# ToddThomson/Mila

Hardware: AMD Instinct MI355X
Metric: Gemma-4 12B decode tok/s (B=1, context 2048), 1xMI355X (higher is better)
Workload: dtype bf16; 1 GPU; Gemma-4 12B, weight policy bf16, B=1, prefill T=2048 then decode at positions 2048..; decode_mode=graph, replicas=1, parallelism=replicas only (no collective), bounded_local_kv=0

## Files before the change

include/mila_cdna4.h:

```cpp
#ifndef MILA_CDNA4_H
#define MILA_CDNA4_H

#include <stddef.h>
#include <stdint.h>

#ifdef __cplusplus
extern "C" {
#endif

#if defined(__GNUC__)
#define MILA_API __attribute__((visibility("default")))
#else
#define MILA_API
#endif

typedef void* mila_stream_t;

enum {
    MILA_OK = 0,
    MILA_E_INVALID_ARGUMENT = -1,
    MILA_E_UNSUPPORTED = -2,
    MILA_E_RUNTIME = -3,
    MILA_E_SCRATCH_TOO_SMALL = -4
};
// ... 215 lines not shown
    int* argmax_blocks;
} mila_fused_matvec_args;
MILA_API int mila_cdna4_fused_norm_matvec(const mila_fused_matvec_args* host_args, mila_stream_t stream);

MILA_API int mila_cdna4_fused_qkv_post(uint16_t* q_out, uint16_t* Kc, uint16_t* Vc, const uint16_t* q,
                                       const uint16_t* k, const uint16_t* v_src, const uint16_t* qw,
                                       const uint16_t* kw, const uint16_t* vw, const float* cos_cache,
                                       const float* sin_cache, int NH, int NKV, int HS, int position,
                                       int capacity, float eps, mila_stream_t stream);


MILA_API int mila_cdna4_fused_qkv_post_prefill(uint16_t* q_out, uint16_t* Kc, uint16_t* Vc, const uint16_t* q,
                                               const uint16_t* k, const uint16_t* v_src, int64_t src_row_stride,
                                               const uint16_t* qw, const uint16_t* kw, const uint16_t* vw,
                                               const float* cos_cache, const float* sin_cache, int T, int NH, int NKV,
                                               int HS, int pos_offset, int capacity, float eps, mila_stream_t stream);
MILA_API int mila_cdna4_fused_tail_norm_bf16(uint16_t* R, uint16_t* XN, const uint16_t* A, const uint16_t* RES,
                                             const uint16_t* post_w, const uint16_t* next_w, int rows, int dim,
                                             float post_scale, float eps, mila_stream_t stream);
MILA_API int mila_cdna4_fused_tail_norm_quant_bf16(uint16_t* R, uint16_t* XN, uint8_t* XQ, float* XS, const uint16_t* A,
                                                   const uint16_t* RES, const uint16_t* post_w, const uint16_t* next_w, int rows,
                                                   int dim, float post_scale, float eps, mila_stream_t stream);

MILA_API int mila_cdna4_attn_decode_bf16_devpos(uint16_t* Y, const uint16_t* Q, const uint16_t* Kc,
                                                const uint16_t* Vc, void* scratch, size_t scratch_bytes,
                                                int B, int NH, int NKV, int HS, int capacity,
                                                const int32_t* position_dev, int max_len, int window,
                                                float scale, mila_stream_t stream);
MILA_API int mila_cdna4_fused_qkv_post_devpos(uint16_t* q_out, uint16_t* Kc, uint16_t* Vc, const uint16_t* q,
                                              const uint16_t* k, const uint16_t* v_src, const uint16_t* qw,
                                              const uint16_t* kw, const uint16_t* vw, const float* cos_cache,
                                              const float* sin_cache, int NH, int NKV, int HS,
                                              const int32_t* position_dev, int capacity, float eps,
                                              mila_stream_t stream);
MILA_API int mila_cdna4_advance_position(int32_t* position_dev, mila_stream_t stream);
MILA_API int mila_cdna4_advance_position_snapshot(int32_t* position_dev, const int32_t* token, unsigned long long* seq_dev, unsigned long long* ring, int ring_size,
                                                  mila_stream_t stream);
MILA_API int mila_cdna4_snapshot_token(const int32_t* token, unsigned long long* seq_dev, unsigned long long* ring, int ring_size, mila_stream_t stream);
MILA_API int mila_cdna4_sample_argmax_advance_fp32(const float* logits, int32_t* token_out, int vocab, void* scratch, size_t scratch_bytes,
                                                   int32_t* position_dev, unsigned long long* seq_dev, unsigned long long* ring, int ring_size,
                                                   mila_stream_t stream);

MILA_API int mila_cdna4_sample_argmax_final_advance(int32_t* token_out, const void* scratch, size_t scratch_bytes, int blocks, int32_t* position_dev,
                                                    unsigned long long* seq_dev, unsigned long long* ring, int ring_size, mila_stream_t stream);

MILA_API int mila_cdna4_fused_attn_decode_bf16(uint16_t* Y, uint16_t* Kc, uint16_t* Vc, const uint16_t* q_raw,
                                               const uint16_t* k_raw, const uint16_t* v_raw, const uint16_t* qw,
                                               const uint16_t* kw, const uint16_t* vw, const float* cos_cache,
                                               const float* sin_cache, void* scratch, size_t scratch_bytes, int NH,
                                               int NKV, int HS, int capacity, int position,
                                               const int32_t* position_dev, int window, float scale, float eps,
                                               mila_stream_t stream);

MILA_API int mila_cdna4_fused_attn_decode_batch_bf16(uint16_t* Y, uint16_t* Kc, uint16_t* Vc, const uint16_t* q_raw, const uint16_t* k_raw,
                                                     const uint16_t* v_raw, int64_t raw_b_stride, const uint16_t* qw, const uint16_t* kw,
                                                     const uint16_t* vw, const float* cos_cache, const float* sin_cache, void* scratch,
                                                     size_t scratch_bytes, int B, int NH, int NKV, int HS, int capacity, int position,
                                                     const int32_t* position_dev, int window, float scale, float eps, mila_stream_t stream);

#ifdef __cplusplus
}
#endif
#endif
```

mila_amd/capi.py:

```python
import ctypes as C
import os

_HERE = os.path.dirname(os.path.abspath(__file__))
LIB_PATH = os.path.join(_HERE, "lib", "libmila_cdna4.so")

MILA_OK = 0
MILA_E_INVALID_ARGUMENT = -1
MILA_E_UNSUPPORTED = -2
MILA_E_RUNTIME = -3
MILA_E_SCRATCH_TOO_SMALL = -4

FMT_BF16, FMT_FP8, FMT_FP4 = 0, 1, 2


class MilaError(RuntimeError):
    def __init__(self, code, text):
        super().__init__("mila_cdna4 error %d: %s" % (code, text))
        self.code = code


class InvalidArgument(MilaError, ValueError):
    """reference: std::invalid_argument"""


# ... 104 lines not shown
    lib = load()
    lib.mila_cdna4_gemm_plan_describe.restype = C.c_size_t
    buf = C.create_string_buffer(8192)
    need = lib.mila_cdna4_gemm_plan_describe(PLAN_ENTRIES.index(entry) if isinstance(entry, str) else int(entry), int(M), int(K), int(N), buf, C.c_size_t(len(buf)))
    assert need <= len(buf), "plan text of %d bytes" % need
    return [(f[0],) + tuple(int(v) for v in f[1:]) for f in (item.split(":") for item in buf.value.decode().split("+") if item)]


def check(rc):
    if rc == MILA_OK:
        return
    text = load().mila_cdna4_last_error().decode()
    if rc == MILA_E_INVALID_ARGUMENT:
        raise InvalidArgument(rc, text)
    raise MilaError(rc, text)


def call(name, *args):
    fn = getattr(load(), "mila_cdna4_" + name)
    conv = []
    for a in args:
        if a is None or isinstance(a, (C.c_void_p, C.c_float, C.c_int, C.c_int64, C.c_size_t)):
            conv.append(a)
        elif isinstance(a, float):
            conv.append(C.c_float(a))
        elif isinstance(a, int):
            conv.append(C.c_int(a))
        elif hasattr(a, "data_ptr"):
            conv.append(_ptr(a))
        else:
            conv.append(a)
    check(fn(*conv, _stream()))


EXPORTED = [
    "last_error", "abi_version", "device_count", "set_device", "device_info", "stream_create",
    "stream_destroy", "stream_synchronize", "malloc", "free", "host_alloc_pinned", "host_free_pinned",
    "memcpy_h2d", "memcpy_d2h", "memcpy_d2d", "memset_zero",
    "matvec_bf16", "matvec_bf16_qfp8", "matvec_bf16_qfp4", "matvec_f32out",
    "gemm_bf16", "gemm_gelu_bf16", "gemm_workspace_bytes", "gemm_bf16_ws", "gemm_bf16_w8a16", "gemm_bf16_w4a16", "gemm_staging_bytes", "gemm_bf16_w8a16_staged", "gemm_bf16_w4a16_staged",
    "fp4_weight_fp8_scale", "upcast_fp4_to_fp8", "quantize_fp8_per_token", "gemm_fp8_applicable", "gemm_fp8_scaled", "gemm_fp8_workspace_bytes", "gemm_fp8_scaled_ws",
    "gemm_w4a8_scratch_bytes", "gemm_bf16_w4a8", "gemm_geglu_w4a8_applicable", "gemm_geglu_bf16_w4a8",
    "gemm_geglu_applicable", "gemm_geglu_preferred", "gemm_geglu_bf16", "gemm_geglu_bf16_w8a16_staged", "gemm_geglu_bf16_w4a16_staged",
    "quantize_fp8_per_channel", "quantize_fp4_per_group",
    "kv_write_bf16", "attn_decode_scratch_bytes", "attn_decode_bf16", "attn_prefill_bf16", "mha_bf16", "mha_kv_write_bf16", "mha_decode_scratch_bytes", "mha_decode_bf16",
    "rmsnorm_bf16", "rmsnorm_fp32", "layernorm_bf16", "layernorm_fp32", "softmax_fp32", "softmax_bf16",
    "gelu_bf16", "gelu_fp32", "geglu_bf16", "residual_bf16", "residual_fp32",
    "rope_build_cache", "rope_forward_bf16",
    "embedding_gather_bf16", "embedding_gather_bf16_qfp8", "lpe_bf16", "split3_bf16", "scale_bf16",
    "convert_f32_to_bf16", "convert_bf16_to_f32", "fill_uniform_bf16",
    "sample_scratch_bytes", "sample_argmax_fp32", "sample_argmax_bf16",
    "sample_stochastic_scratch_bytes", "sample_stochastic_fp32", "sample_stochastic_bf16",
    "fused_norm_matvec", "fused_qkv_post", "fused_qkv_post_prefill", "fused_tail_norm_bf16", "fused_tail_norm_quant_bf16",
    "attn_decode_bf16_devpos", "fused_qkv_post_devpos", "advance_position", "advance_position_snapshot", "snapshot_token", "sample_argmax_advance_fp32", "sample_argmax_final_advance", "fused_attn_decode_batch_bf16", "fused_attn_decode_bf16",
    "dequantize_to_bf16", "gemm_geglu_fp8_scaled",
    "gemm_fp8_w8a8_ws", "gemm_geglu_fp8_w8a8", "gemm_w8a8_scratch_bytes", "gemm_bf16_w8a8", "gemm_geglu_bf16_w8a8",
    "matvec_fp32", "gemm_fp32", "mha_fp32", "mha_kv_write_fp32", "mha_decode_fp32", "lpe_fp32", "rope_forward_fp32",
]

INTERNAL = [
    "tune", "tune_get", "tune_reset", "tune_list", "last_form", "gemm_plan_describe",
    "decode_engine_debug",
    "selftest_decode", "selftest_wave_reduce", "selftest_mfma_fp8", "stream_copy", "stream_read",
    "attn_decode_split_count", "fused_attn_decode_partials_bf16", "matvec_attn_combine",
    "decode_chain_scratch_bytes", "decode_chain_init", "decode_chain_status", "decode_chain",
    "decode_engine_scratch_bytes", "decode_engine_init", "decode_engine_status", "decode_engine_applicable", "decode_engine",
    "attn_decode_ticket_count", "fused_attn_decode_onepass_bf16", "prefetch_l3", "fused_attn_decode_ex",
    "exp_gemm4w_bf16", "exp_gemm4w_geglu_bf16",
]
EXPERIMENTS_LIB = [
    "decode_chain_scratch_bytes", "decode_chain_init", "decode_chain_status", "decode_chain",
    "decode_engine_scratch_bytes", "decode_engine_init", "decode_engine_status", "decode_engine_applicable", "decode_engine", "decode_engine_debug",
    "exp_gemm4w_bf16", "exp_gemm4w_geglu_bf16",
]
```

mila_amd/csrc/attention.hip:

```cpp
#include "common.h"
#include "rms_common.h"
#include "rope_common.h"
#include "internal.h"
#include "attention_generic.h"
#include "attention_tiles.h"

namespace mila {

constexpr int kMaxSplits = 64;
constexpr int kMaxSplitsMfma = 256;
constexpr int kMfmaMinBand = 8192;
static int g_mfma_min_band = kMfmaMinBand;
MILA_TUNE("attn.mfma_min_band", g_mfma_min_band);

__global__ __launch_bounds__(256) void kv_write_bf16_kernel(uint16_t* __restrict__ Kc, uint16_t* __restrict__ Vc,
                                                            const uint16_t* __restrict__ k,
                                                            const uint16_t* __restrict__ v, int64_t total_vec,
                                                            int chunk, int NKV, int HS, int start_pos, int capacity)
{
    const int hv = HS / 8;
    const int64_t stride = (int64_t)gridDim.x * 256;
    for (int64_t i = (int64_t)blockIdx.x * 256 + threadIdx.x; i < total_vec; i += stride)
    {
        const int e = (int)(i % hv);
// ... 1018 lines not shown
}

size_t mila_cdna4_mha_decode_scratch_bytes(int B, int C, int NH)
{
    if (B <= 0 || C <= 0 || NH <= 0 || C % NH != 0) return 0;
    return mila_cdna4_attn_decode_scratch_bytes(B, NH, C / NH);
}

int mila_cdna4_mha_decode_bf16(uint16_t* Y, const uint16_t* QKV, uint16_t* Kc, uint16_t* Vc, void* scratch, size_t scratch_bytes, int B, int C,
                               int NH, int capacity, int position, mila_stream_t stream)
{
    MILA_REQUIRE(Y && QKV && Kc && Vc, "mha_decode_bf16: null pointer");
    MILA_REQUIRE(B > 0 && C > 0 && NH > 0 && C % NH == 0 && capacity > 0, "mha_decode_bf16: bad sizes (B=%d C=%d NH=%d capacity=%d)", B, C, NH, capacity);
    MILA_REQUIRE(position >= 0 && position < capacity, "mha_decode_bf16: position %d out of range [0, %d)", position, capacity);
    const int HS = C / NH;
    int rc = mila_cdna4_mha_kv_write_bf16(Kc, Vc, QKV, B, 1, C, NH, position, capacity, stream);
    if (rc) return rc;
    return run_decode_q(Y, QKV, 3 * (int64_t)C, Kc, Vc, scratch, scratch_bytes, B, NH, NH, HS, capacity, position, 0, 1.0f / sqrtf((float)HS),
                        "mha_decode_bf16", as_stream(stream));
}

int mila_cdna4_attn_decode_split_count(int B, int NH, int NKV, int HS, int capacity, int window)
{
    if (B <= 0 || NH <= 0 || NKV <= 0 || NH % NKV != 0 || capacity <= 0 || window < 0) return 0;
    const int band_max = (window > 0 && window < capacity) ? window : capacity;
    return decode_splits(B, NH, NKV, HS, band_max);
}

int mila_cdna4_fused_attn_decode_partials_bf16(uint16_t* Kc, uint16_t* Vc, const uint16_t* q_raw, const uint16_t* k_raw,
                                               const uint16_t* v_raw, const uint16_t* qw, const uint16_t* kw, const uint16_t* vw,
                                               const float* cos_cache, const float* sin_cache, void* scratch, size_t scratch_bytes,
                                               int NH, int NKV, int HS, int capacity, int position, const int32_t* position_dev,
                                               int window, float scale, float eps, mila_stream_t stream)
{
    MILA_REQUIRE(Kc && Vc && q_raw && k_raw && v_raw && qw && kw && cos_cache && sin_cache, "fused_attn_decode_partials_bf16: null pointer");
    MILA_REQUIRE(NH > 0 && NKV > 0 && NH % NKV == 0, "fused_attn_decode_partials_bf16: bad head counts (NH=%d NKV=%d)", NH, NKV);
    MILA_REQUIRE(capacity > 0 && window >= 0 && (position_dev || position >= 0), "fused_attn_decode_partials_bf16: bad sizes");
    MILA_REQUIRE(HS % 16 == 0, "fused_attn_decode_partials_bf16: HS=%d must be a multiple of 16", HS);
    MILA_REQUIRE(mila_cdna4_attn_decode_split_count(1, NH, NKV, HS, capacity, window) > 1,
                 "fused_attn_decode_partials_bf16: this (window, capacity) runs unsplit; use fused_attn_decode_bf16");
    if (!position_dev)
    {
        const int len = position + 1, band = (window > 0 && window < len) ? window : len;
        MILA_REQUIRE(band <= capacity, "fused_attn_decode_partials_bf16: live band %d exceeds the cache capacity %d", band, capacity);
    }
    AttnParams f{};
    f.q_raw = q_raw; f.k_raw = k_raw; f.v_raw = v_raw; f.qw = qw; f.kw = kw; f.vw = vw; f.cos_cache = cos_cache; f.sin_cache = sin_cache;
    f.eps = eps;
    f.no_combine = 1;
    return run_decode(nullptr, nullptr, Kc, Vc, scratch, scratch_bytes, 1, NH, NKV, HS, capacity, position, position_dev, window, scale, &f,
                      "fused_attn_decode_partials_bf16", as_stream(stream));
}

size_t mila_cdna4_attn_decode_ticket_count(int B, int NH)
{
    if (B <= 0 || NH <= 0) return 0;
    return (size_t)B * NH;
}

int mila_cdna4_fused_attn_decode_onepass_bf16(uint16_t* Y, uint16_t* Kc, uint16_t* Vc, const uint16_t* q_raw, const uint16_t* k_raw,
                                              const uint16_t* v_raw, const uint16_t* qw, const uint16_t* kw, const uint16_t* vw,
                                              const float* cos_cache, const float* sin_cache, void* scratch, size_t scratch_bytes,
                                              uint32_t* tickets, size_t ticket_count, int NH, int NKV, int HS, int capacity, int position,
                                              const int32_t* position_dev, int window, float scale, float eps, mila_stream_t stream)
{
    MILA_REQUIRE(Y && Kc && Vc && q_raw && k_raw && v_raw && qw && kw && cos_cache && sin_cache && tickets, "fused_attn_decode_onepass_bf16: null pointer");
    MILA_REQUIRE(NH > 0 && NKV > 0 && NH % NKV == 0, "fused_attn_decode_onepass_bf16: bad head counts (NH=%d NKV=%d)", NH, NKV);
    MILA_REQUIRE(capacity > 0 && window >= 0 && (position_dev || position >= 0), "fused_attn_decode_onepass_bf16: bad sizes");
    MILA_REQUIRE(HS % 16 == 0, "fused_attn_decode_onepass_bf16: HS=%d must be a multiple of 16", HS);
    MILA_REQUIRE(ticket_count >= mila_cdna4_attn_decode_ticket_count(1, NH), "fused_attn_decode_onepass_bf16: %zu tickets < required %zu",
                 ticket_count, mila_cdna4_attn_decode_ticket_count(1, NH));
    if (!position_dev)
    {
        const int len = position + 1, band = (window > 0 && window < len) ? window : len;
        MILA_REQUIRE(band <= capacity, "fused_attn_decode_onepass_bf16: live band %d exceeds the cache capacity %d", band, capacity);
    }
    AttnParams f{};
    f.q_raw = q_raw; f.k_raw = k_raw; f.v_raw = v_raw; f.qw = qw; f.kw = kw; f.vw = vw; f.cos_cache = cos_cache; f.sin_cache = sin_cache;
    f.eps = eps;
    f.tickets = tickets;
    return run_decode(Y, nullptr, Kc, Vc, scratch, scratch_bytes, 1, NH, NKV, HS, capacity, position, position_dev, window, scale, &f,
                      "fused_attn_decode_onepass_bf16", as_stream(stream));
}

int mila_cdna4_fused_attn_decode_ex(const mila_fused_attn_args* a, mila_stream_t stream)
{
    MILA_REQUIRE(a != nullptr, "fused_attn_decode_ex: null arguments");
    MILA_REQUIRE(a->Y && a->Kc && a->Vc && a->q_raw && a->k_raw && a->v_raw && a->qw && a->kw && a->cos_cache && a->sin_cache, "fused_attn_decode_ex: null pointer");
    MILA_REQUIRE(a->NH > 0 && a->NKV > 0 && a->NH % a->NKV == 0, "fused_attn_decode_ex: bad head counts (NH=%d NKV=%d)", a->NH, a->NKV);
    MILA_REQUIRE(a->capacity > 0 && a->window >= 0 && (a->position_dev || a->position >= 0), "fused_attn_decode_ex: bad sizes");
    MILA_REQUIRE(a->HS % 16 == 0, "fused_attn_decode_ex: HS=%d must be a multiple of 16", a->HS);
    MILA_REQUIRE(a->warm_a_blocks >= 0 && a->warm_a_blocks <= 64 && a->warm_b_blocks >= 0 && a->warm_b_blocks <= 64, "fused_attn_decode_ex: warm block counts must be in [0, 64]");
    if (a->tickets)
        MILA_REQUIRE(a->ticket_count >= mila_cdna4_attn_decode_ticket_count(1, a->NH), "fused_attn_decode_ex: %zu tickets < required %zu",
                     a->ticket_count, mila_cdna4_attn_decode_ticket_count(1, a->NH));
    if (!a->position_dev)
    {
        const int len = a->position + 1, band = (a->window > 0 && a->window < len) ? a->window : len;
        MILA_REQUIRE(band <= a->capacity, "fused_attn_decode_ex: live band %d exceeds the cache capacity %d", band, a->capacity);
    }
    AttnParams f{};
    f.q_raw = a->q_raw; f.k_raw = a->k_raw; f.v_raw = a->v_raw; f.qw = a->qw; f.kw = a->kw; f.vw = a->vw; f.cos_cache = a->cos_cache; f.sin_cache = a->sin_cache;
    f.eps = a->eps;
    f.tickets = a->tickets;
    if (a->warm_a && a->warm_a_bytes >= 128 && a->warm_a_blocks > 0) { f.warm_a = (const uint8_t*)a->warm_a; f.warm_a_lines = (int64_t)(a->warm_a_bytes / 128); f.warm_a_blocks = a->warm_a_blocks; }
    if (a->warm_b && a->warm_b_bytes >= 128 && a->warm_b_blocks > 0) { f.warm_b = (const uint8_t*)a->warm_b; f.warm_b_lines = (int64_t)(a->warm_b_bytes / 128); f.warm_b_blocks = a->warm_b_blocks; f.warm_b_pair = (int64_t)a->warm_b_pair_offset; }
// ... 6 lines not shown
```

mila_amd/csrc/matvec.hip:

```cpp
#include <cstdio>
#include <cstdlib>

#include "common.h"
#include "internal.h"
#include "rms_common.h"
#include "matvec_body.h"

namespace mila {

template <int FMT, int R, int U, int PRO, bool GEGLU, bool F32OUT, int XC, int XSRC = X_PLAIN>
__global__ __launch_bounds__(1024) void matvec_kernel(const MatvecParams p)
{
    extern __shared__ __attribute__((aligned(16))) unsigned char smem_raw[];
    __shared__ float red_a[16 * XC], red_b[16 * XC];
    u32x4 rkeep[XC];
    matvec_body<FMT, R, U, PRO, GEGLU, F32OUT ? Y_F32 : Y_BF16, XC, XSRC, RES_MEM>(
        p, reinterpret_cast<u32x4*>(smem_raw), red_a, red_b, (int)blockIdx.x, (int)gridDim.x, rkeep, NoWait{});
}

static int g_tune_R = 0, g_tune_U = 0, g_tune_blocks = 0;
MILA_TUNE("matvec.rows_per_wave", g_tune_R);
MILA_TUNE("matvec.chunks_in_flight", g_tune_U);
MILA_TUNE("matvec.max_workgroups", g_tune_blocks);
static thread_local int t_last_matvec_blocks = 0;
// ... 33 lines not shown
    ShapeOverrides o;
    const char* env = getenv("MILA_MATVEC_SHAPE");
    if (!env) return o;
    int f, t, r, u, b, n = 0;
    while (*env && sscanf(env, "f%dt%d=%d,%d,%d%n", &f, &t, &r, &u, &b, &n) == 5)
    {
        if (f >= 0 && f < 3 && t >= 0 && t < 3 && r >= 1 && u >= 1 && b >= 1) { o.e[f][t].set = true; o.e[f][t].rows = r; o.e[f][t].U = u; o.e[f][t].blocks = b; }
        env += n;
        if (*env == ';') ++env;
    }
    return o;
}

template <int FMT, int PRO, bool GEGLU, bool F32OUT>
static int dispatch_RU(const MatvecParams& p, hipStream_t s)
{
    const int rows = GEGLU ? 2 * p.N : p.N;
    const bool tall = rows >= 16384, huge = rows >= 100000;
    int rows_per_step, U;
    if (FMT == FMT_BF16) { rows_per_step = huge ? 4 : (tall ? 2 : 1); U = tall ? 2 : 4; }
    else if (FMT == FMT_FP8) { rows_per_step = huge ? 4 : (tall ? 2 : 1); U = 2; }
    else { rows_per_step = tall ? 2 : 1; U = huge ? 2 : 1; }
    int max_blocks = (huge || (tall && FMT == FMT_BF16)) ? 2 * kNumCU : kNumCU;
    {
        static const ShapeOverrides ov = parse_shape_overrides();
        const ShapeOverrides::E& e = ov.e[FMT][huge ? 2 : (tall ? 1 : 0)];
        if (e.set) { rows_per_step = e.rows; U = e.U; max_blocks = e.blocks; }
    }
    int R = GEGLU ? (rows_per_step >= 2 ? rows_per_step / 2 : 1) : rows_per_step;
    if (g_tune_R > 0) R = g_tune_R;
    if (g_tune_U > 0) U = g_tune_U;
    if (g_tune_blocks > 0) max_blocks = g_tune_blocks;
    if (p.amax_v && max_blocks > kArgmaxPartials) max_blocks = kArgmaxPartials;
    if (GEGLU && R > 2) R = 2;
    if (R == 1 && U == 1) return launch<FMT, 1, 1, PRO, GEGLU, F32OUT>(p, max_blocks, s);
    if (R == 1 && U == 2) return launch<FMT, 1, 2, PRO, GEGLU, F32OUT>(p, max_blocks, s);
    if (R == 1) return launch<FMT, 1, 4, PRO, GEGLU, F32OUT>(p, max_blocks, s);
    if (R == 2 && U == 1) return launch<FMT, 2, 1, PRO, GEGLU, F32OUT>(p, max_blocks, s);
    if (R == 2) return launch<FMT, 2, 2, PRO, GEGLU, F32OUT>(p, max_blocks, s);
    if constexpr (!GEGLU) return launch<FMT, 4, 2, PRO, GEGLU, F32OUT>(p, max_blocks, s);
    return launch<FMT, 2, 2, PRO, GEGLU, F32OUT>(p, max_blocks, s);
}

template <int FMT, int U, int XSRC>
static int launch_combine_t(const MatvecParams& p, hipStream_t s)
{
    constexpr int EPC = Fmt<FMT>::kElemsPerChunk;
    const int nchunks = p.K / EPC;
    const int S = (nchunks + 64 * U - 1) / (64 * U);
    const size_t lds = (size_t)S * 64 * U * EPC * 2;
    MILA_REQUIRE(lds <= 65536, "matvec_attn_combine: K=%d needs %zu bytes of LDS for x (limit 65536)", p.K, lds);
    int blocks = (p.N + kMatvecWaves - 1) / kMatvecWaves;
    if (blocks > kNumCU) blocks = kNumCU;
    hipLaunchKernelGGL((matvec_kernel<FMT, 1, U, 0, false, false, 1, XSRC>), dim3(blocks), dim3(64 * kMatvecWaves), lds, s, p);
    MILA_LAUNCH_CHECK("matvec_attn_combine");
}
template <int XSRC>
static int launch_combine(int fmt, const MatvecParams& p, hipStream_t s)
{
    switch (fmt)
    {
        case FMT_BF16: return launch_combine_t<FMT_BF16, 4, XSRC>(p, s);
        case FMT_FP8: return launch_combine_t<FMT_FP8, 2, XSRC>(p, s);
        default: return launch_combine_t<FMT_FP4, 1, XSRC>(p, s);
    }
}

static int validate(const char* who, const void* y, const void* x, const void* W, const float* scales,
                    int fmt, int K, int N, int group)
{
    MILA_REQUIRE(y && x && W, "%s: null pointer (y=%p x=%p W=%p)", who, y, x, W);
    MILA_REQUIRE(K > 0 && N > 0, "%s: K and N must be positive (K=%d N=%d)", who, K, N);
    MILA_REQUIRE(K <= 16384, "%s: K=%d exceeds the register-staged x limit (16384)", who, K);
    if (fmt == FMT_BF16) MILA_REQUIRE(K % 8 == 0, "%s: K=%d must be a multiple of 8 for bf16 weights", who, K);
    if (fmt == FMT_FP8)
    {
        MILA_REQUIRE(K % 16 == 0, "%s: K=%d must be a multiple of 16 for fp8 weights", who, K);
        MILA_REQUIRE(scales != nullptr, "%s: fp8 weights need per-channel scales", who);
    }
    if (fmt == FMT_FP4)
    {
        MILA_REQUIRE(group == 64 || group == 128, "%s: fp4 group size must be 64 or 128 (got %d)", who, group);
        MILA_REQUIRE(K % 32 == 0 && K % group == 0, "%s: K=%d must be a multiple of 32 and of the group size %d", who, K, group);
        MILA_REQUIRE(scales != nullptr, "%s: fp4 weights need per-group scales", who);
    }
    MILA_REQUIRE(fmt >= 0 && fmt <= 2, "%s: unknown weight format %d", who, fmt);
    return MILA_OK;
}

template <int PRO, bool GEGLU, bool F32OUT>
static int dispatch_fmt(int fmt, const MatvecParams& p, hipStream_t s)
{
    switch (fmt)
    {
        case FMT_BF16: return dispatch_RU<FMT_BF16, PRO, GEGLU, F32OUT>(p, s);
        case FMT_FP8: return dispatch_RU<FMT_FP8, PRO, GEGLU, F32OUT>(p, s);
        default: return dispatch_RU<FMT_FP4, PRO, GEGLU, F32OUT>(p, s);
    }
}

}

using namespace mila;

extern "C" {

int mila_cdna4_matvec_bf16(uint16_t* y, const uint16_t* x, const uint16_t* W, const uint16_t* bias, int K,
                           int N, mila_stream_t stream)
{
    int rc = validate("matvec_bf16", y, x, W, nullptr, FMT_BF16, K, N, 0);
    if (rc) return rc;
    MatvecParams p{y, x, reinterpret_cast<const uint8_t*>(W), nullptr, bias, nullptr, nullptr, nullptr, nullptr, 1.0f, 0.0f, K, N, 0, 0, 0};
    return dispatch_fmt<0, false, false>(FMT_BF16, p, as_stream(stream));
}

int mila_cdna4_matvec_bf16_qfp8(uint16_t* y, const uint16_t* x, const uint8_t* W, const float* scales,
                                const uint16_t* bias, int K, int N, mila_stream_t stream)
{
    int rc = validate("matvec_bf16_qfp8", y, x, W, scales, FMT_FP8, K, N, 0);
    if (rc) return rc;
    MatvecParams p{y, x, W, scales, bias, nullptr, nullptr, nullptr, nullptr, 1.0f, 0.0f, K, N, 0, 0, 0};
    return dispatch_fmt<0, false, false>(FMT_FP8, p, as_stream(stream));
}

int mila_cdna4_matvec_bf16_qfp4(uint16_t* y, const uint16_t* x, const uint8_t* W_packed, const float* scales,
                                const uint16_t* bias, int K, int N, int group, mila_stream_t stream)
{
    int rc = validate("matvec_bf16_qfp4", y, x, W_packed, scales, FMT_FP4, K, N, group);
    if (rc) return rc;
    MatvecParams p{y, x, W_packed, scales, bias, nullptr, nullptr, nullptr, nullptr, 1.0f, 0.0f, K, N, group, 0, 0};
    return dispatch_fmt<0, false, false>(FMT_FP4, p, as_stream(stream));
}

int mila_cdna4_matvec_f32out(float* y, const uint16_t* x, const void* W, const float* scales, int fmt, int K,
                             int N, int group, mila_stream_t stream)
{
    int rc = validate("matvec_f32out", y, x, W, scales, fmt, K, N, group);
    if (rc) return rc;
    MatvecParams p{y, x, reinterpret_cast<const uint8_t*>(W), scales, nullptr, nullptr, nullptr, nullptr, nullptr, 1.0f, 0.0f, K, N, group, 0, 0};
    return dispatch_fmt<0, false, true>(fmt, p, as_stream(stream));
}

int mila_cdna4_matvec_attn_combine(uint16_t* y, const void* partials, int splits, int NH, int HS, const void* W, const float* scales,
                                   int fmt, int N, int group, mila_stream_t stream)
{
    MILA_REQUIRE(partials != nullptr, "matvec_attn_combine: null partials");
    MILA_REQUIRE(HS == 256 || HS == 512, "matvec_attn_combine: head size %d must be 256 or 512 (a wave's 64 chunks span 2 or 1 heads)", HS);
    MILA_REQUIRE(NH > 0 && splits > 1 && splits <= 64, "matvec_attn_combine: need NH > 0 and 1 < splits <= 64 (NH=%d splits=%d)", NH, splits);
    const int K = NH * HS;
    MILA_REQUIRE(K <= 8192, "matvec_attn_combine: NH * HS = %d exceeds 8192", K);
    int rc = validate("matvec_attn_combine", y, partials, W, scales, fmt, K, N, group);
    if (rc) return rc;
    MatvecParams p{y, reinterpret_cast<const uint16_t*>(partials), reinterpret_cast<const uint8_t*>(W), scales, nullptr, nullptr, nullptr, nullptr,
                   nullptr, 1.0f, 0.0f, K, N, group, splits, NH};
    return HS == 512 ? launch_combine<X_COMBINE_1>(fmt, p, as_stream(stream)) : launch_combine<X_COMBINE_2>(fmt, p, as_stream(stream));
}

int mila_cdna4_fused_norm_matvec(const mila_fused_matvec_args* a, mila_stream_t stream)
{
    MILA_REQUIRE(a != nullptr, "fused_norm_matvec: null args");
    const int rows = a->geglu ? 2 * a->N : a->N;
    (void)rows;
    int rc = validate("fused_norm_matvec", a->y, a->x, a->W, a->scales, a->fmt, a->K, a->N, a->group);
    if (rc) return rc;
    MILA_REQUIRE(a->norm_w != nullptr, "fused_norm_matvec: norm_w is required");
    MILA_REQUIRE((a->res == nullptr) == (a->post_w == nullptr), "fused_norm_matvec: res and post_w go together");
    if (a->res)
    {
        MILA_REQUIRE(a->res_out != nullptr, "fused_norm_matvec: res_out is required with res");
        MILA_REQUIRE(a->res_out != a->res && a->res_out != a->x, "fused_norm_matvec: res_out must not alias res or x");
    }
    MatvecParams p{a->y, a->x, reinterpret_cast<const uint8_t*>(a->W), a->scales, nullptr, a->norm_w, a->post_w,
                   a->res, a->res_out, a->post_scale, a->eps, a->K, a->N, a->group, 0, 0};
    hipStream_t s = as_stream(stream);
    MILA_REQUIRE(!(a->geglu && a->f32_out), "fused_norm_matvec: geglu and f32_out are exclusive");
    if (a->argmax_scratch)
    {
        MILA_REQUIRE(a->f32_out, "fused_norm_matvec: argmax_scratch needs f32_out (the logits)");
        MILA_REQUIRE(a->argmax_blocks != nullptr, "fused_norm_matvec: argmax_blocks is required with argmax_scratch");
        if (a->argmax_scratch_bytes < mila_cdna4_sample_scratch_bytes())
            return set_error(MILA_E_SCRATCH_TOO_SMALL, "fused_norm_matvec: argmax scratch %zu bytes < required %zu", a->argmax_scratch_bytes, mila_cdna4_sample_scratch_bytes());
        p.amax_v = reinterpret_cast<float*>(a->argmax_scratch);
        p.amax_i = reinterpret_cast<int*>(p.amax_v + kArgmaxPartials);
    }
    if (a->f32_out)
    {
        rc = a->res ? dispatch_fmt<2, false, true>(a->fmt, p, s) : dispatch_fmt<1, false, true>(a->fmt, p, s);
        if (rc == MILA_OK && a->argmax_scratch)
        {
            if (t_last_matvec_blocks > kArgmaxPartials) return set_error(MILA_E_RUNTIME, "fused_norm_matvec: %d workgroups exceed the %d sampler partials", t_last_matvec_blocks, kArgmaxPartials);
            *a->argmax_blocks = t_last_matvec_blocks;
        }
        return rc;
    }
    if (a->res)
        return a->geglu ? dispatch_fmt<2, true, false>(a->fmt, p, s) : dispatch_fmt<2, false, false>(a->fmt, p, s);
    return a->geglu ? dispatch_fmt<1, true, false>(a->fmt, p, s) : dispatch_fmt<1, false, false>(a->fmt, p, s);
}

}
```

mila_amd/csrc/matvec_body.h:

```cpp
#pragma once
#include "common.h"
#include "rms_common.h"

namespace mila {

enum { FMT_BF16 = 0, FMT_FP8 = 1, FMT_FP4 = 2 };

template <int FMT> struct Fmt;
template <> struct Fmt<FMT_BF16> { static constexpr int kElemsPerChunk = 8; };
template <> struct Fmt<FMT_FP8> { static constexpr int kElemsPerChunk = 16; };
template <> struct Fmt<FMT_FP4> { static constexpr int kElemsPerChunk = 32; };

template <int FMT>
__device__ __forceinline__ float chunk_dot(const u32x4 w, const u32x4* __restrict__ xs, int c, float acc)
{
    if constexpr (FMT == FMT_BF16)
    {
        const u32x4 xv = xs[c];
#pragma unroll
        for (int d = 0; d < 4; ++d) acc = dot2_bf16(as_bf16x2(w[d]), as_bf16x2(xv[d]), acc);
    }
    else if constexpr (FMT == FMT_FP8)
    {
        const u32x4 x0 = xs[2 * c], x1 = xs[2 * c + 1];
// ... 101 lines not shown
    constexpr int EPC = Fmt<FMT>::kElemsPerChunk;
    constexpr int XPC = EPC / 8;
    constexpr int NR = GEGLU ? 2 * R : R;
    const int nchunks = K / EPC;
    const size_t row_bytes = (size_t)nchunks * 16;
    const int S = (nchunks + 64 * U - 1) / (64 * U);
    const int nx16_pad = S * 64 * U * XPC;
    const int ngroups = (FMT == FMT_FP4) ? K / p.group : 0;
    const int cpg_shift = (FMT == FMT_FP4) ? (p.group == 128 ? 2 : 1) : 0;
    const int total_waves = nblocks * kMatvecWaves;
    const int n_rg = (N + R - 1) / R;
    const int wave_g = block * kMatvecWaves + wib;
    const int nrg_w = wave_g < n_rg ? (n_rg - 1 - wave_g) / total_waves + 1 : 0;
    const int T = nrg_w * S;

    u32x4 px[XC], pnw[PRO != 0 ? XC : 1], ppw[PRO == 2 ? XC : 1], pres[PRO == 2 ? XC : 1];
#pragma unroll
    for (int k = 0; k < XC; ++k)
    {
        const size_t e = (size_t)min(tid + 1024 * k, nx16 - 1) * 8;
        if constexpr (XSRC == X_PLAIN) px[k] = ld16(p.x + e);
        if constexpr (PRO != 0) pnw[k] = ld16(p.norm_w + e);
        if constexpr (PRO == 2)
        {
            ppw[k] = ld16(p.post_w + e);
            if constexpr (RSRC == RES_MEM) pres[k] = ld16(p.res + e);
            else pres[k] = rkeep[k];
        }
    }

    auto issue = [&](WBuf<FMT, U, NR>& b, int rg, int s) {
        const int c0 = s * (64 * U) + lane;
#pragma unroll
        for (int j = 0; j < NR; ++j)
        {
            const int col = min(rg * R + (GEGLU ? (j >> 1) : j), N - 1);
            const int row = (GEGLU && (j & 1)) ? (N + col) : col;
            const uint8_t* wrow = p.W + (size_t)row * row_bytes;
#pragma unroll
            for (int u = 0; u < U; ++u)
            {
                const int c = min(c0 + 64 * u, nchunks - 1);
                b.w[u][j] = ld16_nt(wrow + (size_t)c * 16);
                if constexpr (FMT == FMT_FP4) b.sc[u][j] = p.scales[(size_t)row * ngroups + (c >> cpg_shift)];
            }
        }
    };
    int ci_rg = wave_g, ci_s = 0, cc_rg = wave_g, cc_s = 0;
    auto advance = [&](int& rg_, int& s_) {
        const bool wrap = (s_ + 1 == S);
        s_ = wrap ? 0 : s_ + 1;
        rg_ = wrap ? rg_ + total_waves : rg_;
    };
    WBuf<FMT, U, NR> ba, bb;
    issue(ba, ci_rg, ci_s); advance(ci_rg, ci_s);
    issue(bb, ci_rg, ci_s); advance(ci_rg, ci_s);

    if constexpr (XSRC == X_COMBINE_1 || XSRC == X_COMBINE_2)
    {
        constexpr int HPW = (XSRC == X_COMBINE_1) ? 1 : 2;
        const float* part = reinterpret_cast<const float*>(p.x);
        const int splits = p.comb_splits, HS = 512 / HPW, STR = HS + 4;
#pragma unroll
        for (int k = 0; k < XC; ++k)
        {
            const int c = tid + 1024 * k;
            const int h0 = ((c & ~63) * 8) / HS;
            const int myj = (HPW == 1) ? 0 : (lane >> 5);
            float fs[HPW], Lh[HPW];
#pragma unroll
            for (int j = 0; j < HPW; ++j)
            {
                const int h = min(h0 + j, p.comb_heads - 1);
                const float* hb = part + (size_t)h * splits * STR;
                const float ms = (lane < splits) ? hb[(size_t)lane * STR + HS] : -INFINITY;
                const float ls = (lane < splits) ? hb[(size_t)lane * STR + HS + 1] : 0.0f;
                const float M = wave_max(ms);
                fs[j] = (ms == -INFINITY) ? 0.0f : __expf(ms - M);
                Lh[j] = wave_sum(ls * fs[j]);
            }
            const int h = min(h0 + myj, p.comb_heads - 1);
            const float* vb = part + (size_t)h * splits * STR + (size_t)((c * 8) % HS);
            float acc[8];
#pragma unroll
            for (int e = 0; e < 8; ++e) acc[e] = 0.0f;
            for (int s0 = 0; s0 < splits; s0 += 8)
            {
                f32x4 va[8], vb2[8];
#pragma unroll
                for (int u = 0; u < 8; ++u)
                {
                    const float* src = vb + (size_t)min(s0 + u, splits - 1) * STR;
                    va[u] = *reinterpret_cast<const f32x4*>(src);
                    vb2[u] = *reinterpret_cast<const f32x4*>(src + 4);
                }
#pragma unroll
                for (int u = 0; u < 8; ++u)
                {
                    const int si = min(s0 + u, 63);
                    float f = __uint_as_float(__builtin_amdgcn_readlane(__float_as_uint(fs[0]), si));
                    if constexpr (HPW == 2)
                    {
                        const float f1 = __uint_as_float(__builtin_amdgcn_readlane(__float_as_uint(fs[1]), si));
                        f = myj ? f1 : f;
                    }
                    if (s0 + u >= splits) f = 0.0f;
#pragma unroll
                    for (int e = 0; e < 4; ++e)
                    {
                        acc[e] = fmaf(va[u][e], f, acc[e]);
                        acc[4 + e] = fmaf(vb2[u][e], f, acc[4 + e]);
                    }
                }
            }
            float L = Lh[0];
            if constexpr (HPW == 2) L = myj ? Lh[1] : Lh[0];
#pragma unroll
            for (int d = 0; d < 4; ++d)
                px[k][d] = pack_bf16x2(L > 0.0f ? acc[2 * d] / L : 0.0f, L > 0.0f ? acc[2 * d + 1] / L : 0.0f);
        }
    }

    wait();
    if constexpr (XSRC == X_HANDOFF)
    {
#pragma unroll
        for (int k = 0; k < XC; ++k)
            px[k] = handoff_load8(reinterpret_cast<const uint32_t*>(p.x), min(tid + 1024 * k, nx16 - 1));
    }

    for (int i = nx16 + tid; i < nx16_pad; i += 1024) xs[i] = u32x4{0u, 0u, 0u, 0u};
    if constexpr (PRO == 0)
    {
#pragma unroll
        for (int k = 0; k < XC; ++k)
            if (tid + 1024 * k < nx16) xs[tid + 1024 * k] = px[k];
    }
    else
    {
        const int G = (nx16 + 63) / 64;
        auto rstd_of = [&](const u32x4* v, float* red) {
#pragma unroll
            for (int k = 0; k < XC; ++k)
            {
                float s = (tid + 1024 * k < nx16) ? sumsq8(v[k], 0.0f) : 0.0f;
                s = wave_sum(s);
                if (lane == 0) red[wib + kMatvecWaves * k] = s;
            }
            __syncthreads();
            float t = 0.0f;
            for (int g = 0; g < G; ++g) t += red[g];
            return rsqrtf(t / (float)K + p.eps);
        };
        if constexpr (PRO == 1)
        {
            const float rstd = rstd_of(px, red_a);
#pragma unroll
            for (int k = 0; k < XC; ++k)
                if (tid + 1024 * k < nx16) xs[tid + 1024 * k] = rms_apply8(px[k], pnw[k], rstd, 0.0f);
        }
        else
        {
            const float rstd_a = rstd_of(px, red_a);
#pragma unroll
            for (int k = 0; k < XC; ++k) rkeep[k] = sandwich_tail8(rms_apply8(px[k], ppw[k], rstd_a, 0.0f), pres[k], p.post_scale);
            if (block == 0 && p.res_out != nullptr)
            {
#pragma unroll
                for (int k = 0; k < XC; ++k)
                    if (tid + 1024 * k < nx16) st16(p.res_out + (size_t)(tid + 1024 * k) * 8, rkeep[k]);
            }
            const float rstd_r = rstd_of(rkeep, red_b);
#pragma unroll
            for (int k = 0; k < XC; ++k)
                if (tid + 1024 * k < nx16) xs[tid + 1024 * k] = rms_apply8(rkeep[k], pnw[k], rstd_r, 0.0f);
        }
    }
    __syncthreads();

    float acc[NR];
#pragma unroll
    for (int j = 0; j < NR; ++j) acc[j] = 0.0f;

    auto compute = [&](const WBuf<FMT, U, NR>& b, int s) {
#pragma unroll
// ... 106 lines not shown
```

mila_amd/host/include/Mila/Gemma.h:

```cpp
#pragma once
#include <functional>
#include <map>

#include <hip/hip_runtime_api.h>

#include <algorithm>
#include <cmath>

#include "GemmaBlock.h"
#include "Serialization.h"

namespace Mila::Dnn
{
    struct GemmaConfig
    {
        dim_t vocab_size = 262144, embedding_dim = 3840, num_layers = 48, num_heads = 16, num_kv_heads = 8, head_dim = 256,
              hidden_dim = 15360, global_head_dim = 512, num_global_kv_heads = 1, window = 1024, sliding_window_pattern = 6,
              global_rotary_dim = 128;
        float rms_norm_eps = 1e-6f, rope_theta_local = 10000.0f, rope_theta_global = 1000000.0f, final_logit_softcapping = 30.0f;
        bool bounded_local_kv = false;

        bool isGlobalLayer( dim_t i ) const { return ( i + 1 ) % sliding_window_pattern == 0; }
        dim_t headDim( bool g ) const { return g ? global_head_dim : head_dim; }
        dim_t numKvHeads( bool g ) const { return g ? num_global_kv_heads : num_kv_heads; }
// ... 690 lines not shown
        {
            mila_fused_matvec_args a{};
            a.y = y; a.x = x; a.W = lin.getWeight().rawData();
            a.scales = nullptr;
            if constexpr ( TWeightQuant::kIsQuantized ) a.scales = lin.getWeightScale()->data();
            a.post_scale = 1.0f; a.eps = cfg_.rms_norm_eps; a.fmt = kFmt; a.K = (int)lin.getConfig().getInputFeatures();
            a.N = (int)lin.getConfig().getOutputFeatures(); a.group = Quant::Weight::groupSizeOf<TWeightQuant>(); a.geglu = 0;
            return a;
        }
        void plainMatvec( LinearType& lin, uint16_t* y, const uint16_t* x )
        {
            auto in = TensorType();
            (void)in;
            const int K = (int)lin.getConfig().getInputFeatures(), N = (int)lin.getConfig().getOutputFeatures();
            mila_stream_t st = ctx_->getStream();
            if constexpr ( kFmt == 0 ) Compute::rocmCheck( mila_cdna4_matvec_bf16( y, x, static_cast<const uint16_t*>( lin.getWeight().rawData() ), nullptr, K, N, st ) );
            else if constexpr ( kFmt == 1 ) Compute::rocmCheck( mila_cdna4_matvec_bf16_qfp8( y, x, static_cast<const uint8_t*>( lin.getWeight().rawData() ), lin.getWeightScale()->data(), nullptr, K, N, st ) );
            else Compute::rocmCheck( mila_cdna4_matvec_bf16_qfp4( y, x, static_cast<const uint8_t*>( lin.getWeight().rawData() ), lin.getWeightScale()->data(), nullptr, K, N,
                                                                  Quant::Weight::groupSizeOf<TWeightQuant>(), st ) );
        }
        void fusedGateUp( Layer& L )
        {
            auto a = baseArgs( *L.fc_gate_up, f_act_->data(), f_o_->data() );
            a.N = (int)cfg_.hidden_dim; a.geglu = 1;
            a.norm_w = L.pre_ffn_norm->getWeight()->data(); a.post_w = L.post_attn_norm->getWeight()->data();
            a.res = cur_hidden_; a.res_out = res1_->data();
            Compute::rocmCheck( mila_cdna4_fused_norm_matvec( &a, ctx_->getStream() ) );
        }

        void enqueueFusedStep( const int32_t* token_dev, int position, const int32_t* pos_dev, int* sampler_partials = nullptr )
        {
            mila_stream_t st = ctx_->getStream();
            embed( token_dev, 1, *hidden_[ 0 ] );
            cur_hidden_ = hidden_[ 0 ]->data();
            int next = 1;
            const Layer* prev = nullptr;
            for ( auto& L : layers_ )
            {
                const bool g = L.global;
                const int NH = (int)cfg_.num_heads, NKV = (int)cfg_.numKvHeads( g ), HD = (int)cfg_.headDim( g );
                auto a = baseArgs( *L.qkv_proj, f_qkv_->data(), prev ? f_down_->data() : cur_hidden_ );
                a.norm_w = L.input_norm->getWeight()->data();
                if ( prev )
                {
                    a.post_w = prev->post_ffn_norm->getWeight()->data(); a.res = res1_->data(); a.res_out = hidden_[ next ]->data(); a.post_scale = prev->layer_scalar;
                }
                Compute::rocmCheck( mila_cdna4_fused_norm_matvec( &a, st ) );
                if ( prev ) { cur_hidden_ = hidden_[ next ]->data(); next = ( next == 1 ) ? 2 : 1; }
                const uint16_t* qp = f_qkv_->data();
                const uint16_t* kp = qp + (size_t)NH * HD;
                const uint16_t* vp = g ? kp : kp + (size_t)NKV * HD;
                const size_t need = attnScratchBytes();
                void* scratch = attn_partials_->data();
                Compute::rocmCheck( mila_cdna4_fused_attn_decode_bf16( attn_out_->data(), L.keyCache(), L.valueCache(), qp, kp, vp, L.q_norm->getWeight()->data(),
                                                                       L.k_norm->getWeight()->data(), L.v_norm->getWeight()->data(), L.rope->cosCache(), L.rope->sinCache(),
                                                                       scratch, need, NH, NKV, HD, (int)L.cacheCapacity(), position, pos_dev,
                                                                       (int)cfg_.windowFor( g ), L.attentionScale(), cfg_.rms_norm_eps, st ) );
                plainMatvec( *L.o_proj, f_o_->data(), attn_out_->data() );
                fusedGateUp( L );
                plainMatvec( *L.fc_down, f_down_->data(), f_act_->data() );
                prev = &L;
            }
            {
                mila_fused_matvec_args a{};
                a.y = reinterpret_cast<uint16_t*>( logits_->data() ); a.x = f_down_->data(); a.W = lm_head_->getWeight().rawData();
                a.scales = nullptr;
                if constexpr ( kTableFmt != 0 ) a.scales = lm_head_->getWeightScale()->data();
                a.norm_w = final_norm_->getWeight()->data(); a.post_w = prev->post_ffn_norm->getWeight()->data();
                a.res = res1_->data(); a.res_out = hidden_[ next ]->data(); a.post_scale = prev->layer_scalar; a.eps = cfg_.rms_norm_eps;
                a.fmt = kTableFmt; a.K = (int)cfg_.embedding_dim; a.N = (int)cfg_.vocab_size; a.group = 0; a.geglu = 0; a.f32_out = 1;
                if ( sampler_partials ) { a.argmax_scratch = sample_scratch_->data(); a.argmax_scratch_bytes = sample_scratch_->sizeInBytes(); a.argmax_blocks = sampler_partials; }
                Compute::rocmCheck( mila_cdna4_fused_norm_matvec( &a, st ) );
            }
        }

    public:
        static const char* weightQuantizationName() { return kFmt == 0 ? "none" : kFmt == 1 ? "per_channel_fp8_e4m3" : "per_group_fp4_128"; }

        Serialization::PretrainedMetadata pretrainedMetadata() const
        {
            Serialization::PretrainedMetadata m;
            m.architecture = "gemma4"; m.model_name = name_;
            m.vocab_size = (uint32_t)cfg_.vocab_size; m.max_seq_length = (uint32_t)max_seq_; m.embedding_dim = (uint32_t)cfg_.embedding_dim; m.num_layers = (uint32_t)cfg_.num_layers;
            m.num_heads = (uint32_t)cfg_.num_heads; m.num_kv_heads = (uint32_t)cfg_.num_kv_heads; m.head_dim = (uint32_t)cfg_.head_dim; m.hidden_dim = (uint32_t)cfg_.hidden_dim;
            m.use_bias = false; m.tie_word_embeddings = true; m.activation = "gelu"; m.norm_type = "rmsnorm"; m.attention_type = "gqa"; m.positional_encoding = "rope";
            m.rope_theta = cfg_.rope_theta_local; m.norm_epsilon = cfg_.rms_norm_eps;
            m.global_head_dim = (uint32_t)cfg_.global_head_dim; m.num_global_kv_heads = (uint32_t)cfg_.num_global_kv_heads; m.key_equals_value = true;
            m.window = (uint32_t)cfg_.window; m.sliding_window_pattern = (uint32_t)cfg_.sliding_window_pattern; m.global_rotary_dim = (uint32_t)cfg_.global_rotary_dim;
            m.rope_theta_local = cfg_.rope_theta_local; m.rope_theta_global = cfg_.rope_theta_global; m.final_logit_softcapping = cfg_.final_logit_softcapping;
            return m;
        }

    private:
        struct SaveItem { std::string name, dtype; std::vector<int64_t> shape; const void* dev; size_t bytes; float host_scalar; };
        std::vector<SaveItem> saveItems()
        {
            std::vector<SaveItem> items;
            auto shapeOf = []( const auto& t ) { std::vector<int64_t> v; for ( auto d : t.shape() ) v.push_back( (int64_t)d ); return v; };
            auto storageName = []( auto& lin )
            {
                using L = std::remove_reference_t<decltype( lin )>;
                if constexpr ( !L::kIsQuantized ) return "BF16"; else return L::kWeightDtype == TensorDataType::FP8_E4M3 ? "F8_E4M3" : "U8";
            };
            auto addLinear = [&]( auto& lin, const std::string& flat, const char* wname, const char* sname )
            {
                auto& w = lin.getWeight();
                items.push_back( { flat + "." + wname, storageName( lin ), shapeOf( w ), w.rawData(), w.sizeInBytes(), 0.0f } );
                if constexpr ( std::remove_reference_t<decltype( lin )>::kIsQuantized )
                    items.push_back( { flat + "." + sname, "F32", shapeOf( *lin.getWeightScale() ), lin.getWeightScale()->rawData(), lin.getWeightScale()->sizeInBytes(), 0.0f } );
            };
            auto addNorm = [&]( RmsNormType& n ) { items.push_back( { flatName( n.getName() ) + ".weight", "BF16", shapeOf( *n.getWeight() ), n.getWeight()->rawData(), n.getWeight()->sizeInBytes(), 0.0f } ); };
// ... 267 lines not shown
```

Measured before the change: 223.7 tok/s.

## Fold split-KV attention combine into the o_proj matvec prologue for decode

Adds a fused attention-decode plus o_proj entry point. On windowed local layers with multiple splits, it writes attention partials and merges them inside the o_proj matvec's x-loading prologue. This removes the separate combine pass and the round trip of attn_out through memory. The combine prologue is reworked to process 4-float quads with 16-split prefetching issued before the weight loads, overlapping partial reads with weight streaming. Global layers and unsplit cases fall back to the old attention kernel followed by a plain matvec.

```diff
diff --git a/include/mila_cdna4.h b/include/mila_cdna4.h
--- a/include/mila_cdna4.h
+++ b/include/mila_cdna4.h
@@ -291,6 +291,13 @@
                                                const int32_t* position_dev, int window, float scale, float eps,
                                                mila_stream_t stream);
 
+MILA_API int mila_cdna4_fused_attn_decode_o_proj(uint16_t* y, uint16_t* attn_out, uint16_t* Kc, uint16_t* Vc, const uint16_t* q_raw,
+                                                 const uint16_t* k_raw, const uint16_t* v_raw, const uint16_t* qw, const uint16_t* kw,
+                                                 const uint16_t* vw, const float* cos_cache, const float* sin_cache, void* scratch,
+                                                 size_t scratch_bytes, int NH, int NKV, int HS, int capacity, int position,
+                                                 const int32_t* position_dev, int window, float scale, float eps, const void* W_o,
+                                                 const float* scales_o, int fmt, int N, int group, mila_stream_t stream);
+
 MILA_API int mila_cdna4_fused_attn_decode_batch_bf16(uint16_t* Y, uint16_t* Kc, uint16_t* Vc, const uint16_t* q_raw, const uint16_t* k_raw,
                                                      const uint16_t* v_raw, int64_t raw_b_stride, const uint16_t* qw, const uint16_t* kw,
                                                      const uint16_t* vw, const float* cos_cache, const float* sin_cache, void* scratch,
diff --git a/mila_amd/capi.py b/mila_amd/capi.py
--- a/mila_amd/capi.py
+++ b/mila_amd/capi.py
@@ -180,7 +180,7 @@
     "sample_scratch_bytes", "sample_argmax_fp32", "sample_argmax_bf16",
     "sample_stochastic_scratch_bytes", "sample_stochastic_fp32", "sample_stochastic_bf16",
     "fused_norm_matvec", "fused_qkv_post", "fused_qkv_post_prefill", "fused_tail_norm_bf16", "fused_tail_norm_quant_bf16",
-    "attn_decode_bf16_devpos", "fused_qkv_post_devpos", "advance_position", "advance_position_snapshot", "snapshot_token", "sample_argmax_advance_fp32", "sample_argmax_final_advance", "fused_attn_decode_batch_bf16", "fused_attn_decode_bf16",
+    "attn_decode_bf16_devpos", "fused_qkv_post_devpos", "advance_position", "advance_position_snapshot", "snapshot_token", "sample_argmax_advance_fp32", "sample_argmax_final_advance", "fused_attn_decode_batch_bf16", "fused_attn_decode_bf16", "fused_attn_decode_o_proj",
     "dequantize_to_bf16", "gemm_geglu_fp8_scaled",
     "gemm_fp8_w8a8_ws", "gemm_geglu_fp8_w8a8", "gemm_w8a8_scratch_bytes", "gemm_bf16_w8a8", "gemm_geglu_bf16_w8a8",
     "matvec_fp32", "gemm_fp32", "mha_fp32", "mha_kv_write_fp32", "mha_decode_fp32", "lpe_fp32", "rope_forward_fp32",
diff --git a/mila_amd/csrc/attention.hip b/mila_amd/csrc/attention.hip
--- a/mila_amd/csrc/attention.hip
+++ b/mila_amd/csrc/attention.hip
@@ -1094,6 +1094,37 @@
                       "fused_attn_decode_partials_bf16", as_stream(stream));
 }
 
+static int g_fold_combine = 1;
+MILA_TUNE("decode.fold_combine", g_fold_combine);
+
+int mila_cdna4_fused_attn_decode_o_proj(uint16_t* y, uint16_t* attn_out, uint16_t* Kc, uint16_t* Vc, const uint16_t* q_raw, const uint16_t* k_raw,
+                                        const uint16_t* v_raw, const uint16_t* qw, const uint16_t* kw, const uint16_t* vw, const float* cos_cache,
+                                        const float* sin_cache, void* scratch, size_t scratch_bytes, int NH, int NKV, int HS, int capacity, int position,
+                                        const int32_t* position_dev, int window, float scale, float eps, const void* W_o, const float* scales_o, int fmt,
+                                        int N, int group, mila_stream_t stream)
+{
+    MILA_REQUIRE(y && attn_out && W_o, "fused_attn_decode_o_proj: null pointer");
+    MILA_REQUIRE(NH > 0 && NKV > 0 && NH % NKV == 0 && HS > 0, "fused_attn_decode_o_proj: bad head counts (NH=%d NKV=%d HS=%d)", NH, NKV, HS);
+    MILA_REQUIRE(capacity > 0 && window >= 0 && N > 0, "fused_attn_decode_o_proj: bad sizes");
+    MILA_REQUIRE(fmt >= 0 && fmt <= 2, "fused_attn_decode_o_proj: unknown weight format %d", fmt);
+    const bool windowed = window > 0 && window < capacity;
+    const int splits = windowed ? decode_splits(1, NH, NKV, HS, window) : 1;
+    if (g_fold_combine && windowed && splits > 1 && (HS == 256 || HS == 512) && NH * HS <= 8192)
+    {
+        int rc = mila_cdna4_fused_attn_decode_partials_bf16(Kc, Vc, q_raw, k_raw, v_raw, qw, kw, vw, cos_cache, sin_cache, scratch, scratch_bytes, NH, NKV, HS, capacity,
+                                                            position, position_dev, window, scale, eps, stream);
+        if (rc) return rc;
+        return mila_cdna4_matvec_attn_combine(y, scratch, splits, NH, HS, W_o, scales_o, fmt, N, group, stream);
+    }
+    int rc = mila_cdna4_fused_attn_decode_bf16(attn_out, Kc, Vc, q_raw, k_raw, v_raw, qw, kw, vw, cos_cache, sin_cache, scratch, scratch_bytes, NH, NKV, HS, capacity,
+                                               position, position_dev, window, scale, eps, stream);
+    if (rc) return rc;
+    const int K = NH * HS;
+    if (fmt == 0) return mila_cdna4_matvec_bf16(y, attn_out, reinterpret_cast<const uint16_t*>(W_o), nullptr, K, N, stream);
+    if (fmt == 1) return mila_cdna4_matvec_bf16_qfp8(y, attn_out, reinterpret_cast<const uint8_t*>(W_o), scales_o, nullptr, K, N, stream);
+    return mila_cdna4_matvec_bf16_qfp4(y, attn_out, reinterpret_cast<const uint8_t*>(W_o), scales_o, nullptr, K, N, group, stream);
+}
+
 size_t mila_cdna4_attn_decode_ticket_count(int B, int NH)
 {
     if (B <= 0 || NH <= 0) return 0;
diff --git a/mila_amd/csrc/matvec.hip b/mila_amd/csrc/matvec.hip
--- a/mila_amd/csrc/matvec.hip
+++ b/mila_amd/csrc/matvec.hip
@@ -109,6 +109,7 @@
     MILA_REQUIRE(lds <= 65536, "matvec_attn_combine: K=%d needs %zu bytes of LDS for x (limit 65536)", p.K, lds);
     int blocks = (p.N + kMatvecWaves - 1) / kMatvecWaves;
     if (blocks > kNumCU) blocks = kNumCU;
+    note_form("matvec_attn_combine");
     hipLaunchKernelGGL((matvec_kernel<FMT, 1, U, 0, false, false, 1, XSRC>), dim3(blocks), dim3(64 * kMatvecWaves), lds, s, p);
     MILA_LAUNCH_CHECK("matvec_attn_combine");
 }
@@ -202,7 +203,7 @@
                                    int fmt, int N, int group, mila_stream_t stream)
 {
     MILA_REQUIRE(partials != nullptr, "matvec_attn_combine: null partials");
-    MILA_REQUIRE(HS == 256 || HS == 512, "matvec_attn_combine: head size %d must be 256 or 512 (a wave's 64 chunks span 2 or 1 heads)", HS);
+    MILA_REQUIRE(HS == 256 || HS == 512, "matvec_attn_combine: head size %d must be 256 or 512 (the 256 dims a wave merges lie in one head)", HS);
     MILA_REQUIRE(NH > 0 && splits > 1 && splits <= 64, "matvec_attn_combine: need NH > 0 and 1 < splits <= 64 (NH=%d splits=%d)", NH, splits);
     const int K = NH * HS;
     MILA_REQUIRE(K <= 8192, "matvec_attn_combine: NH * HS = %d exceeds 8192", K);
@@ -210,7 +211,7 @@
     if (rc) return rc;
     MatvecParams p{y, reinterpret_cast<const uint16_t*>(partials), reinterpret_cast<const uint8_t*>(W), scales, nullptr, nullptr, nullptr, nullptr,
                    nullptr, 1.0f, 0.0f, K, N, group, splits, NH};
-    return HS == 512 ? launch_combine<X_COMBINE_1>(fmt, p, as_stream(stream)) : launch_combine<X_COMBINE_2>(fmt, p, as_stream(stream));
+    return K <= 4096 ? launch_combine<X_COMBINE_1>(fmt, p, as_stream(stream)) : launch_combine<X_COMBINE_2>(fmt, p, as_stream(stream));
 }
 
 int mila_cdna4_fused_norm_matvec(const mila_fused_matvec_args* a, mila_stream_t stream)
diff --git a/mila_amd/csrc/matvec_body.h b/mila_amd/csrc/matvec_body.h
--- a/mila_amd/csrc/matvec_body.h
+++ b/mila_amd/csrc/matvec_body.h
@@ -177,72 +177,75 @@
         s_ = wrap ? 0 : s_ + 1;
         rg_ = wrap ? rg_ + total_waves : rg_;
     };
+    constexpr bool COMBINE = (XSRC == X_COMBINE_1 || XSRC == X_COMBINE_2);
+    constexpr int QC = COMBINE ? (XSRC == X_COMBINE_1 ? 1 : 2) : 1;
+    const float* cvb[QC];
+    float cms[QC], cls[QC];
+    f32x4 cv[COMBINE ? 16 : 1];
+    const int csplits = COMBINE ? p.comb_splits : 1, CSTR = COMBINE ? K / p.comb_heads + 4 : 0;
+    auto combine_load = [&](int k, int s0) {
+#pragma unroll
+        for (int u = 0; u < 16; ++u) cv[u] = *reinterpret_cast<const f32x4*>(cvb[k] + (size_t)min(s0 + u, csplits - 1) * CSTR);
+    };
+    if constexpr (COMBINE)
+    {
+        const float* part = reinterpret_cast<const float*>(p.x);
+        const int HS = CSTR - 4, nquads = K / 4;
+#pragma unroll
+        for (int k = 0; k < QC; ++k)
+        {
+            const int q = min(tid + 1024 * k, nquads - 1);
+            const int h = __builtin_amdgcn_readfirstlane((q * 4) / HS);
+            const float* hb = part + (size_t)h * csplits * CSTR;
+            const float* ml = hb + (size_t)min(lane, csplits - 1) * CSTR + HS;
+            cms[k] = ml[0];
+            cls[k] = ml[1];
+            cvb[k] = hb + (q * 4) % HS;
+        }
+        combine_load(0, 0);
+    }
+
     WBuf<FMT, U, NR> ba, bb;
     issue(ba, ci_rg, ci_s); advance(ci_rg, ci_s);
     issue(bb, ci_rg, ci_s); advance(ci_rg, ci_s);
 
-    if constexpr (XSRC == X_COMBINE_1 || XSRC == X_COMBINE_2)
-    {
-        constexpr int HPW = (XSRC == X_COMBINE_1) ? 1 : 2;
-        const float* part = reinterpret_cast<const float*>(p.x);
-        const int splits = p.comb_splits, HS = 512 / HPW, STR = HS + 4;
-#pragma unroll
-        for (int k = 0; k < XC; ++k)
-        {
-            const int c = tid + 1024 * k;
-            const int h0 = ((c & ~63) * 8) / HS;
-            const int myj = (HPW == 1) ? 0 : (lane >> 5);
-            float fs[HPW], Lh[HPW];
-#pragma unroll
-            for (int j = 0; j < HPW; ++j)
-            {
-                const int h = min(h0 + j, p.comb_heads - 1);
-                const float* hb = part + (size_t)h * splits * STR;
-                const float ms = (lane < splits) ? hb[(size_t)lane * STR + HS] : -INFINITY;
-                const float ls = (lane < splits) ? hb[(size_t)lane * STR + HS + 1] : 0.0f;
-                const float M = wave_max(ms);
-                fs[j] = (ms == -INFINITY) ? 0.0f : __expf(ms - M);
-                Lh[j] = wave_sum(ls * fs[j]);
-            }
-            const int h = min(h0 + myj, p.comb_heads - 1);
-            const float* vb = part + (size_t)h * splits * STR + (size_t)((c * 8) % HS);
-            float acc[8];
-#pragma unroll
-            for (int e = 0; e < 8; ++e) acc[e] = 0.0f;
-            for (int s0 = 0; s0 < splits; s0 += 8)
-            {
-                f32x4 va[8], vb2[8];
-#pragma unroll
-                for (int u = 0; u < 8; ++u)
+    if constexpr (COMBINE)
+    {
+        const int nquads = K / 4, n8 = (csplits + 7) & ~7;
+#pragma unroll
+        for (int k = 0; k < QC; ++k)
+        {
+            const float ms = (lane < csplits) ? cms[k] : -INFINITY;
+            const float ls = (lane < csplits) ? cls[k] : 0.0f;
+            const float M = wave_max(ms);
+            const float fs = (ms == -INFINITY) ? 0.0f : __expf(ms - M);
+            const float L = wave_sum(ls * fs);
+            float acc[4] = {0.0f, 0.0f, 0.0f, 0.0f};
+            auto fma16 = [&](int s0) {
+#pragma unroll
+                for (int u = 0; u < 16; ++u)
                 {
-                    const float* src = vb + (size_t)min(s0 + u, splits - 1) * STR;
-                    va[u] = *reinterpret_cast<const f32x4*>(src);
-                    vb2[u] = *reinterpret_cast<const f32x4*>(src + 4);
-                }
-#pragma unroll
-                for (int u = 0; u < 8; ++u)
-                {
-                    const int si = min(s0 + u, 63);
-                    float f = __uint_as_float(__builtin_amdgcn_readlane(__float_as_uint(fs[0]), si));
-                    if constexpr (HPW == 2)
+                    const float f = __uint_as_float(__builtin_amdgcn_readlane(__float_as_uint(fs), min(s0 + u, 63)));
+                    if (s0 + u < n8)
                     {
-                        const float f1 = __uint_as_float(__builtin_amdgcn_readlane(__float_as_uint(fs[1]), si));
-                        f = myj ? f1 : f;
-                    }
-                    if (s0 + u >= splits) f = 0.0f;
-#pragma unroll
-                    for (int e = 0; e < 4; ++e)
-                    {
-                        acc[e] = fmaf(va[u][e], f, acc[e]);
-                        acc[4 + e] = fmaf(vb2[u][e], f, acc[4 + e]);
+#pragma unroll
+                        for (int e = 0; e < 4; ++e) acc[e] = fmaf(s0 + u < csplits ? cv[u][e] : 0.0f, f, acc[e]);
                     }
                 }
-            }
-            float L = Lh[0];
-            if constexpr (HPW == 2) L = myj ? Lh[1] : Lh[0];
-#pragma unroll
-            for (int d = 0; d < 4; ++d)
-                px[k][d] = pack_bf16x2(L > 0.0f ? acc[2 * d] / L : 0.0f, L > 0.0f ? acc[2 * d + 1] / L : 0.0f);
+            };
+            int s0 = 0;
+            if (k == 0)
+            {
+                fma16(0);
+#pragma unroll
+                for (int u = 0; u < 16; ++u) asm volatile("" ::"v"(cv[u]));
+                s0 = 16;
+            }
+#pragma unroll 1
+            for (; s0 < n8; s0 += 16) { combine_load(k, s0); fma16(s0); }
+            const u32x2 o = u32x2{pack_bf16x2(L > 0.0f ? acc[0] / L : 0.0f, L > 0.0f ? acc[1] / L : 0.0f),
+                                  pack_bf16x2(L > 0.0f ? acc[2] / L : 0.0f, L > 0.0f ? acc[3] / L : 0.0f)};
+            if (tid + 1024 * k < nquads) reinterpret_cast<u32x2*>(xs)[tid + 1024 * k] = o;
         }
     }
 
@@ -255,7 +258,8 @@
     }
 
     for (int i = nx16 + tid; i < nx16_pad; i += 1024) xs[i] = u32x4{0u, 0u, 0u, 0u};
-    if constexpr (PRO == 0)
+    if constexpr (COMBINE) {  }
+    else if constexpr (PRO == 0)
     {
 #pragma unroll
         for (int k = 0; k < XC; ++k)
diff --git a/mila_amd/host/include/Mila/Gemma.h b/mila_amd/host/include/Mila/Gemma.h
--- a/mila_amd/host/include/Mila/Gemma.h
+++ b/mila_amd/host/include/Mila/Gemma.h
@@ -766,11 +766,13 @@
                 const uint16_t* vp = g ? kp : kp + (size_t)NKV * HD;
                 const size_t need = attnScratchBytes();
                 void* scratch = attn_partials_->data();
-                Compute::rocmCheck( mila_cdna4_fused_attn_decode_bf16( attn_out_->data(), L.keyCache(), L.valueCache(), qp, kp, vp, L.q_norm->getWeight()->data(),
-                                                                       L.k_norm->getWeight()->data(), L.v_norm->getWeight()->data(), L.rope->cosCache(), L.rope->sinCache(),
-                                                                       scratch, need, NH, NKV, HD, (int)L.cacheCapacity(), position, pos_dev,
-                                                                       (int)cfg_.windowFor( g ), L.attentionScale(), cfg_.rms_norm_eps, st ) );
-                plainMatvec( *L.o_proj, f_o_->data(), attn_out_->data() );
+                const float* o_scales = nullptr;
+                if constexpr ( TWeightQuant::kIsQuantized ) o_scales = L.o_proj->getWeightScale()->data();
+                Compute::rocmCheck( mila_cdna4_fused_attn_decode_o_proj( f_o_->data(), attn_out_->data(), L.keyCache(), L.valueCache(), qp, kp, vp, L.q_norm->getWeight()->data(),
+                                                                         L.k_norm->getWeight()->data(), L.v_norm->getWeight()->data(), L.rope->cosCache(), L.rope->sinCache(),
+                                                                         scratch, need, NH, NKV, HD, (int)L.cacheCapacity(), position, pos_dev,
+                                                                         (int)cfg_.windowFor( g ), L.attentionScale(), cfg_.rms_norm_eps, L.o_proj->getWeight().rawData(), o_scales,
+                                                                         kFmt, (int)L.o_proj->getConfig().getOutputFeatures(), Quant::Weight::groupSizeOf<TWeightQuant>(), st ) );
                 fusedGateUp( L );
                 plainMatvec( *L.fc_down, f_down_->data(), f_act_->data() );
                 prev = &L;
```

New measurement: 221.0 tok/s. 1.2% lower.
